# tomdbar/naqs-for-quantum-chemistry

Measured on AMD Instinct MI355X. Metric: unique samples/sec through E_loc + log-psi eval (N2, 20 qubits), higher is better.
Workload: dtype f32 network (f16x2-split MFMA, f32-equivalent) / f64 E_loc; 1 GPU; N2 STO-3G (20 qubits, K=2239 Pauli terms, Kxy=378), 10000 unique samples per GPU, 1xMI355X per rank; pipeline=2 independent batches in flight on 2 HIP streams (one handle pair each), batches=4 distinct key sets per rank, rotated every step, input=unique sampled bit-strings (keys) resident in HBM; random-init network, ranks=single process, no process group

## Files before the change

naqs-for-quantum-chemistry_amd/csrc/naqs_logpsi.hip:

```cpp

#include <algorithm>
#include <cstdint>
#include <cstdio>
#include <cstring>
#include <new>
#include <vector>

#include "naqs_common.hpp"
#include "naqs_hash.hpp"
#include "naqs_net.hpp"
#include "naqs_amp_mfma.hpp"
#include "naqs_amp_deep.hpp"
#include "naqs_pack.hpp"

namespace {

using naqs::WAVE;
using naqs::DeviceGuard;
using naqs::ElocFeed;

using naqs::MAXP;
using naqs::MAXL;
using naqs::f32x4;
using naqs::NetDims;
using naqs::amp_partial;
using naqs::amp_finish;

#ifndef NAQS_AMP_TILES
#define NAQS_AMP_TILES 4
#endif
#ifndef NAQS_AMP_SPLIT
#define NAQS_AMP_SPLIT 4
#endif
constexpr int AMP_TILES = NAQS_AMP_TILES;
constexpr int AMP_SPLIT = NAQS_AMP_SPLIT;

__device__ __forceinline__ void amp_body(const NetDims &d, const float *__restrict__ w, int64_t M,
// ... 1051 lines not shown
                v = mfma_h<2>(a[0][rb], b[0][c], v);
                acc[rb][c] = v;
            }
    };
#pragma unroll
    for (int c0 = 0; c0 < NC; c0 += 2) load_b2(0, c0);
    load_a(0, a0);
    int k0 = 0;
    for (; k0 + 64 <= Kh_pad; k0 += 64) {
        load_a(k0 + 32, a1);
#pragma unroll
        for (int c0 = 0; c0 < NC; c0 += 2) {
            __builtin_amdgcn_sched_barrier(0);
            mma2(a0, c0);
            __builtin_amdgcn_sched_barrier(0);
            load_b2(k0 + 32, c0);
        }
        const int kn = min(k0 + 64, Kh_pad - 32);
        load_a(kn, a0);
#pragma unroll
        for (int c0 = 0; c0 < NC; c0 += 2) {
            __builtin_amdgcn_sched_barrier(0);
            mma2(a1, c0);
            __builtin_amdgcn_sched_barrier(0);
            load_b2(kn, c0);
        }
    }
    if (k0 < Kh_pad) {
#pragma unroll
        for (int c0 = 0; c0 < NC; c0 += 2) mma2(a0, c0);
    }
}

#ifndef NAQS_SAVE_NT
#define NAQS_SAVE_NT 1
#endif
__device__ __forceinline__ void save_store(f32x4 *ptr, const f32x4 val) {
#if NAQS_SAVE_NT
    __builtin_nontemporal_store(val, ptr);
#else
    *ptr = val;
#endif
}
template <int RB, bool SAVE, int NCT, int C0>
__device__ __forceinline__ void ws_writeback4(ushort_t *__restrict__ planes, int ldh, f32x4 (&acc)[RB][NCT],
                                              const float (&bvs)[NCT], int col0, int lane, float *__restrict__ save, int save_ld,
                                              int64_t row0, int64_t M, const LayerScale sc) {
    constexpr int BM = RB * 16;
    const int kg = lane >> 4;
    const int plane_stride = BM * ldh;
#pragma unroll
    for (int rb = 0; rb < RB; ++rb)
#pragma unroll
        for (int r = 0; r < 4; ++r) {
            float h[4];
#pragma unroll
            for (int c = 0; c < 4; ++c) h[c] = fmaxf(fmaf(acc[rb][C0 + c][r], sc.c, bvs[C0 + c]), 0.0f);
            const int row = rb * 16 + kg * 4 + r;
            if (SAVE && save != nullptr && row0 + row < M)
                save_store(reinterpret_cast<f32x4 *>(save + (row0 + row) * save_ld + col0),
                           (f32x4){h[0] * sc.isn, h[1] * sc.isn, h[2] * sc.isn, h[3] * sc.isn});
            ushort_t *dst = planes + row * ldh + col0;
            uint32_t a1, a2, b1, b2;
            split2_pair(h[0], h[1], a1, a2);
            split2_pair(h[2], h[3], b1, b2);
            *reinterpret_cast<uint2 *>(dst) = make_uint2(a1, b1);
// ... 22 lines not shown
            __builtin_amdgcn_sched_barrier(0);
            amp_mfma_item<CT>(d, f0, n, ab, lane, outs);
        } else {
            if (na < n && n_last > n) { na = n + 1; amp_mfma_load<CT>(wamp + (size_t)na * pair_elems, lane, f0); }
            __builtin_amdgcn_sched_barrier(0);
            amp_mfma_item<CT>(d, f1, n, ab, lane, outs);
        }
    }
    if (clk != nullptr && blockIdx.x == 0 && lane == 0) clk[wave * 16 + 8] = clock64();
    {
        const int r = aw * WAVE + lane;
        if (do_feed && r < BM && feed.tab != nullptr && row0 + r < M) {
            const uint64_t key = keys[row0 + r];
            if (feed.key_bits == 32) naqs::feed_key<uint32_t>(feed, row0 + r, key);
            else naqs::feed_key<uint64_t>(feed, row0 + r, key);
        }
    }
    __builtin_amdgcn_fence(__ATOMIC_RELEASE, "wavefront");
    __builtin_amdgcn_wave_barrier();
    __builtin_amdgcn_fence(__ATOMIC_ACQUIRE, "wavefront");
    for (int e = q0 * 16 + lane; e < q1 * 16; e += WAVE) {
        const int q = e >> 4, s = e & 15;
        const int n = q / RB, r = (q - n * RB) * 16 + s;
        float o[5];
#pragma unroll
        for (int c = 0; c < 5; ++c) o[c] = s_o[((size_t)n * BM + r) * 8 + c];
        const uint32_t ab = s_ab[r], mask = (1u << n) - 1u;
        const int occ = (int)((ab >> n) & 1u) + 2 * (int)((ab >> (16 + n)) & 1u);
        s_lan[n][r] = naqs::amp_finish(d, n, o, ab & mask, (ab >> 16) & mask, occ);
    }
    if (clk != nullptr && blockIdx.x == 0 && lane == 0) clk[wave * 16 + 15] = clock64();
}

struct WsSplit {
    unsigned long long *xchg; uint32_t tag; const naqs::PollCtl *ctl;
    const int64_t *spec_U; int spec_P;
    naqs::SampleFinishJob fin;
};
constexpr int WS_XCHG_ROWS = 80;

template <int RB, bool SAVE, bool SPLIT = false>
__global__ __launch_bounds__(PH_THREADS) void phase_kernel_ws(const NetDims d, const float *__restrict__ w,
                                                              const ushort_t *__restrict__ wh, int64_t M,
                                                              const uint64_t *__restrict__ keys,
                                                              const float *__restrict__ scratch, float2 *__restrict__ out,
                                                              const ElocFeed feed, const naqs::PhaseSave save,
                                                              const ushort_t *__restrict__ wamp,
                                                              const naqs::PhaseScales *__restrict__ scales, const int flags,
                                                              const WsSplit split) {
    extern __shared__ __attribute__((aligned(16))) ushort_t planes[];
    __shared__ uint32_t s_ab[RB * 16];
    __shared__ float s_lan[MAXP][RB * 16];
    __shared__ __attribute__((aligned(16))) float s_part[WS_MW][RB * 16][4];
    __shared__ float s_recv[SPLIT ? RB * 16 : 1][4];
    constexpr int BM = RB * 16;
    constexpr int FMT = 2, NP = 2;
    constexpr int AW = PH_WAVES - WS_MW;
    const int tid = threadIdx.x, lane = tid & 63, wave = __builtin_amdgcn_readfirstlane(tid >> 6);
    const int hosted = split.fin.U != nullptr ? 1 : 0;
    if (hosted && blockIdx.x == 0) {
        __shared__ int64_t s_fin[16];
        naqs::sample_finish_body(split.fin, s_fin);
        return;
    }
    const int bx = (int)blockIdx.x - hosted;
    const int n_tiles = SPLIT ? (int)((gridDim.x - hosted) >> 1) : (int)gridDim.x - hosted;
    const bool producer = SPLIT && bx < n_tiles;
    const int tile = SPLIT && !producer ? bx - n_tiles : bx;
    const int64_t row0 = (int64_t)tile * BM;
    if (split.spec_U != nullptr) {
        const int64_t m_dev = split.spec_U[MAXP + 1] != 0 ? 0 : split.spec_U[split.spec_P];
        M = m_dev < M ? m_dev : M;
        if (row0 >= M) return;
    }
    const int P = d.P, ldh = d.ldh;
    float *s_o = reinterpret_cast<float *>(planes + (size_t)NP * BM * ldh);
    const bool ha64 = d.Ha == 64;

    NAQS_MARK(0);
    uint32_t warm0 = 0, warm1 = 0;
    {
        const uint32_t *w0 = reinterpret_cast<const uint32_t *>(wh + d.wh_off[0]);
        const int n_dw = NP * d.N_pad[0] * d.Kh_pad[0] / 2;
        if (tid * 32 < n_dw) warm0 = w0[tid * 32];
        if ((tid + PH_THREADS) * 32 < n_dw) warm1 = w0[(tid + PH_THREADS) * 32];
    }
    static_assert(BM <= WAVE, "the tile's rows are gathered by wave 0");
    uint64_t key = 0ull;
    if (tid < BM && row0 + tid < M) key = keys[row0 + tid];
    const int aw = wave >= WS_MW ? wave - WS_MW : 0;
    const int items = RB * P;
    const int q_split = SPLIT ? (P / 2) * RB : items;
    const int qlo = producer ? q_split : 0, qhi = producer ? items : q_split;
    const int first_pair = (qlo + (qhi - qlo) * aw / AW) / RB;
    AmpFrag<4> f4;
    AmpFrag<2> f2;
    if (wamp != nullptr && wave >= WS_MW) {
        if (ha64) amp_mfma_load<4>(wamp + (size_t)first_pair * amp_mfma_pair_elems(64), lane, f4);
        else amp_mfma_load<2>(wamp + (size_t)first_pair * amp_mfma_pair_elems(32), lane, f2);
    }
    bf16x8 pre[NP][CBT];
    mlp_layer0_fetch<RB, NP>(d, wh + d.wh_off[0], wave, lane, pre);
    if (tid < BM) {
        uint32_t a = 0, b = 0;
#pragma unroll
        for (int k = 0; k < MAXP; ++k) {
            if (k < P) {
                a |= (uint32_t)((key >> d.qa[k]) & 1ull) << k;
                b |= (uint32_t)((key >> d.qb[k]) & 1ull) << k;
            }
        }
        s_ab[tid] = a | (b << 16);
    }
    __syncthreads();
    NAQS_MARK(1);

    const int m = lane & 15, kg = lane >> 4;
    LayerScale sc;
    sc.c = scales->c[0]; sc.sn = scales->sn[0]; sc.isn = scales->isn[0];
    {
        const int N0 = d.N_pad[0], cb0 = wave * CBT;
        float bvs0[CBT];
#pragma unroll
        for (int c = 0; c < CBT; ++c) bvs0[c] = (w + d.b_off[0])[tile_col(cb0 + c, m, N0)] * sc.sn;
        const uint32_t pmask = (1u << (P - 1)) - 1u;
        const int nv = min(max(2 * (P - 1) - 8 * kg, 0), 8) >> 1;
        f32x4 acc0[RB][CBT];
#pragma unroll
        for (int rb = 0; rb < RB; ++rb) {
            const uint32_t ab = s_ab[rb * 16 + m];
// ... 25 lines not shown
                    save.x[(row0 + r) * save.x_ld + k] = set ? 1.0f : -1.0f;
                }
            }
        }
        ws_writeback4<RB, SAVE, CBT, 0>(planes, ldh, acc0, bvs0, (cb0 >> 2) * 64 + 4 * m, lane, producer ? nullptr : save.act[0], save.act_ld[0],
                                        row0, M, sc);
    }
    asm volatile("" ::"v"(warm0), "v"(warm1));
    __syncthreads();
    NAQS_MARK(5);

    sc.c = scales->c[1]; sc.sn = scales->sn[1]; sc.isn = scales->isn[1];
    const int N1 = d.N_pad[1], Kh1 = d.Kh_pad[1];
    if (wave < WS_MW) {
        constexpr int NCT = SPLIT ? WS_NCT / 2 : WS_NCT;
        constexpr int NG = NCT / 4;
        f32x4 acc[RB][NCT];
        float bvs[NCT];
        if (flags & 1) __builtin_amdgcn_s_setprio(1);
#pragma unroll
        for (int rb = 0; rb < RB; ++rb)
#pragma unroll
            for (int c = 0; c < NCT; ++c) acc[rb][c] = (f32x4){0.f, 0.f, 0.f, 0.f};
        const int cb0 = (producer ? WS_MW * NCT : 0) + wave * NCT;
        const float *bias = w + d.b_off[1];
#pragma unroll
        for (int c = 0; c < NCT; ++c) bvs[c] = bias[tile_col(cb0 + c, m, N1)] * sc.sn;
        const ushort_t *a_ptr = planes + m * ldh + 8 * kg, *w_ptr = wh + d.wh_off[1] + (size_t)cb0 * Kh1 * 16 + lane * 8;
        if (flags & 8) {}
#ifdef NAQS_WS_DEBUG
        else if (flags & 16) ws_accumulate<RB, 1, NCT>(a_ptr, ldh, BM * ldh, w_ptr, Kh1, (size_t)N1 * Kh1, acc);
        else if (flags & 32) ws_accumulate<RB, 2, NCT>(a_ptr, ldh, BM * ldh, w_ptr, Kh1, (size_t)N1 * Kh1, acc);
#endif
        else ws_accumulate<RB, 0, NCT>(a_ptr, ldh, BM * ldh, w_ptr, Kh1, (size_t)N1 * Kh1, acc);
        if (flags & 1) __builtin_amdgcn_s_setprio(0);
        NAQS_MARK(9);
        const float *W2 = w + d.w_off[2];
        const int K2 = d.K_pad[2];
        const int g0 = cb0 >> 2;
        f32x4 wv[NG][4];
#pragma unroll
        for (int g = 0; g < NG; ++g)
#pragma unroll
            for (int o = 0; o < 4; ++o) wv[g][o] = *reinterpret_cast<const f32x4 *>(W2 + (size_t)o * K2 + (g0 + g) * 64 + 4 * m);
#pragma unroll
        for (int rb = 0; rb < RB; ++rb)
#pragma unroll
            for (int r = 0; r < 4; ++r) {
                const int row = rb * 16 + kg * 4 + r;
                float po[4] = {0.f, 0.f, 0.f, 0.f};
#pragma unroll
                for (int g = 0; g < NG; ++g) {
                    float h[4];
#pragma unroll
                    for (int c = 0; c < 4; ++c) h[c] = fmaxf(fmaf(acc[rb][4 * g + c][r], sc.c, bvs[4 * g + c]), 0.0f);
                    if (SAVE && save.act[1] != nullptr && row0 + row < M)
                        save_store(reinterpret_cast<f32x4 *>(save.act[1] + (row0 + row) * save.act_ld[1] + (g0 + g) * 64 + 4 * m),
                                   (f32x4){h[0] * sc.isn, h[1] * sc.isn, h[2] * sc.isn, h[3] * sc.isn});
#pragma unroll
                    for (int o = 0; o < 4; ++o)
#pragma unroll
                        for (int c = 0; c < 4; ++c) po[o] = fmaf(h[c], wv[g][o][c], po[o]);
                }
#pragma unroll
                for (int o = 0; o < 4; ++o) {
                    float v = po[o];
                    v += __builtin_bit_cast(float, __builtin_amdgcn_update_dpp(0, __builtin_bit_cast(int, v), 0xB1, 0xF, 0xF, true));
                    v += __builtin_bit_cast(float, __builtin_amdgcn_update_dpp(0, __builtin_bit_cast(int, v), 0x4E, 0xF, 0xF, true));
                    v += __builtin_bit_cast(float, __builtin_amdgcn_update_dpp(0, __builtin_bit_cast(int, v), 0x141, 0xF, 0xF, true));
                    v += __builtin_bit_cast(float, __builtin_amdgcn_update_dpp(0, __builtin_bit_cast(int, v), 0x140, 0xF, 0xF, true));
                    po[o] = v;
                }
                if (m == 0) *reinterpret_cast<f32x4 *>(&s_part[wave][row][0]) = (f32x4){po[0], po[1], po[2], po[3]};
            }
    } else {
        if (flags & 2) __builtin_amdgcn_s_setprio(1);
        if ((flags & 4) || wamp == nullptr) {}
        else if (ha64) ws_amp_work<4, RB>(d, wamp, M, row0, keys, feed, s_ab, s_lan, s_o, f4, aw, lane, save.clk, wave, qlo, qhi, !producer);
        else ws_amp_work<2, RB>(d, wamp, M, row0, keys, feed, s_ab, s_lan, s_o, f2, aw, lane, save.clk, wave, qlo, qhi, !producer);
        if (flags & 2) __builtin_amdgcn_s_setprio(0);
    }
    NAQS_MARK(10);
    __syncthreads();
    NAQS_MARK(6);

    if constexpr (SPLIT) {
        constexpr int TILE_WORDS = BM * 4 + MAXP * BM;
        static_assert(BM <= WS_XCHG_ROWS, "a tile's words must fit the exchange buffer's per-tile share");
        unsigned long long *xw = split.xchg + (size_t)tile * TILE_WORDS;
        const int n_split = q_split / RB, n_amp = wamp != nullptr ? (P - n_split) * BM : 0;
        const unsigned long long tagw = (unsigned long long)split.tag << 32;
        if (producer) {
            for (int x = tid; x < BM * 4 + n_amp; x += PH_THREADS) {
                float v;
                if (x < BM * 4) {
                    const int r = x >> 2, o = x & 3;
                    v = (s_part[0][r][o] + s_part[1][r][o]) + (s_part[2][r][o] + s_part[3][r][o]);
                } else {
                    const int e = x - BM * 4;
                    v = s_lan[n_split + e / BM][e % BM];
                }
                if (!(naqs::poll_drop(split.ctl, naqs::POLL_LOGPSI_SPLIT) && tile == 0 && x == 0))
                    __hip_atomic_store(&xw[x], tagw | __float_as_uint(v), __ATOMIC_RELAXED, __HIP_MEMORY_SCOPE_AGENT);
            }
            return;
        }
        bool ok = true;
        for (int x = tid; x < BM * 4 + n_amp; x += PH_THREADS) {
            unsigned long long word;
            ok = naqs::poll_tagged<2>(&xw[x], split.tag, word, split.ctl, naqs::POLL_LOGPSI_SPLIT, (uint32_t)x) && ok;
// ... 296 lines not shown
    const bool deep = net->amp.deep(), mlp = naqs::has_phase_mlp(net);
    hipDeviceProp_t prop;
    if (hipGetDeviceProperties(&prop, net->device) == hipSuccess) net->cu_count = prop.multiProcessorCount;
    int st = NAQS_OK;
    if (mlp || !deep) st = dev_alloc(&net->d_w, net->w_floats);
    if (st == NAQS_OK && deep) st = dev_alloc(&net->amp.w, net->amp.deep_floats);
    if (!deep) net->amp.w = net->d_w;
    if (st == NAQS_OK && naqs::has_second_set(net)) st = dev_alloc(&net->ph.w, net->ph.deep() ? net->ph.deep_floats : rows_floats(net->ph.d));
    if (st == NAQS_OK && !deep && (d.Ha == 32 || d.Ha == 64 || d.Ha == 128) && (mlp || 2 * (d.P - 1) <= 30))
        st = dev_alloc(&net->d_wamp, (int64_t)d.P * (int64_t)amp_mfma_pair_elems(d.Ha));
    if (st == NAQS_OK && net->family == naqs::Family::COMBINED) st = dev_alloc(&net->d_cflat, net->comb_amp + net->comb_head);
    if (st != NAQS_OK || !mlp) return st;
    st = dev_alloc(&net->d_wh, net->wh_elems);
    if (st != NAQS_OK) return st;
    const int lds_max = 4 * 16 * std::max(d.ld, PH_WAVES * 16) * (int)sizeof(float);
    (void)hipFuncSetAttribute(reinterpret_cast<const void *>(&phase_kernel<1>), hipFuncAttributeMaxDynamicSharedMemorySize, lds_max / 4);
    (void)hipFuncSetAttribute(reinterpret_cast<const void *>(&phase_kernel<2>), hipFuncAttributeMaxDynamicSharedMemorySize, lds_max / 2);
    (void)hipFuncSetAttribute(reinterpret_cast<const void *>(&phase_kernel<3>), hipFuncAttributeMaxDynamicSharedMemorySize, lds_max / 4 * 3);
    (void)hipFuncSetAttribute(reinterpret_cast<const void *>(&phase_kernel<4>), hipFuncAttributeMaxDynamicSharedMemorySize, lds_max);
    const int lds_all = 160 * 1024 - 5 * 1024;
#define NAQS_PH_ATTR(RB, FMT)                                                                                                            \
    (void)hipFuncSetAttribute(reinterpret_cast<const void *>(&phase_kernel_h<RB, false, FMT>), hipFuncAttributeMaxDynamicSharedMemorySize, lds_all); \
    (void)hipFuncSetAttribute(reinterpret_cast<const void *>(&phase_kernel_h<RB, true, FMT>), hipFuncAttributeMaxDynamicSharedMemorySize, lds_all);
    NAQS_PH_ATTR(1, 1) NAQS_PH_ATTR(2, 1) NAQS_PH_ATTR(3, 1)
    NAQS_PH_ATTR(1, 2) NAQS_PH_ATTR(2, 2) NAQS_PH_ATTR(3, 2) NAQS_PH_ATTR(4, 2)
#undef NAQS_PH_ATTR
#define NAQS_WS_ATTR(RB)                                                                                                                 \
    (void)hipFuncSetAttribute(reinterpret_cast<const void *>(&phase_kernel_ws<RB, false>), hipFuncAttributeMaxDynamicSharedMemorySize, lds_all); \
    (void)hipFuncSetAttribute(reinterpret_cast<const void *>(&phase_kernel_ws<RB, true>), hipFuncAttributeMaxDynamicSharedMemorySize, lds_all); \
    (void)hipFuncSetAttribute(reinterpret_cast<const void *>(&phase_kernel_ws<RB, false, true>), hipFuncAttributeMaxDynamicSharedMemorySize, lds_all); \
    (void)hipFuncSetAttribute(reinterpret_cast<const void *>(&phase_kernel_ws<RB, true, true>), hipFuncAttributeMaxDynamicSharedMemorySize, lds_all);
    NAQS_WS_ATTR(1) NAQS_WS_ATTR(2) NAQS_WS_ATTR(3)
#undef NAQS_WS_ATTR
    (void)hipGetLastError();
    st = dev_alloc(&net->d_raw, 1);
    if (st == NAQS_OK) st = dev_alloc(&net->d_scales, 1);
    if (st == NAQS_OK && hipMemset(net->d_raw, 0, sizeof(naqs::PhaseRaw)) != hipSuccess) st = NAQS_ERR_HIP;
    if (st == NAQS_OK) st = dev_alloc(&net->d_sum_words, 8);
    if (st == NAQS_OK && hipMemset(net->d_sum_words, 0, 8 * sizeof(unsigned long long)) != hipSuccess) st = NAQS_ERR_HIP;
    if (st == NAQS_OK && hipDeviceSynchronize() != hipSuccess) st = NAQS_ERR_HIP;
    return st;
}

static int net_build(const naqs_net_config_t *cfg, const naqs::Family family, const int depth, const int device, naqs_net_t **out) {
    int st = net_validate(cfg, family, depth, device);
    if (st != NAQS_OK) return st;
    naqs_net *net = new (std::nothrow) naqs_net();
    if (!net) return NAQS_ERR_NOMEM;
    net->device = device;
    net->cfg = *cfg;
    net->family = family;
    st = net_layout(net, depth);
    if (st != NAQS_OK) { delete net; return st; }
    (void)naqs::poll_handle_create(device, &net->poll);
    net->ctl = net->poll.dev;
    net->shared_gpu = naqs::env_int("NAQS_SHARED_GPU", 0) == 1;
    DeviceGuard guard;
    st = guard.init(device);
    if (st == NAQS_OK) st = net_alloc(net);
    if (st != NAQS_OK) { naqs_net_destroy(net); return st; }
    *out = net;
    return NAQS_OK;
}

NAQS_API int naqs_net_create(const naqs_net_config_t *cfg, int device, naqs_net_t **out) {
    if (!cfg || !out) return NAQS_ERR_INVALID;
// ... 469 lines not shown
        const ElocFeed none{};
        if (prof) { st = net->prof.begin(s); if (st != NAQS_OK) return st; }
        st = launch_amp_kernel(net->ph.d, net->ph.w, M, keys_dev, s_ph, none, 1, s);
        if (st != NAQS_OK) return st;
        if (prof) { st = net->prof.end(s); if (st != NAQS_OK) return st; }
    }
    NAQS_KLAUNCH(agg_finish_kernel, dim3((unsigned)((M + 255) / 256)), dim3(256), 0, s, net->amp.d.P, M, net->d_scratch, s_ph,
                       reinterpret_cast<float2 *>(logpsi_dev), feed);
    HIP_TRY(hipGetLastError());
    return NAQS_OK;
}

static int comb_logpsi(naqs_net *net, int64_t M, const uint64_t *keys_dev, float *logpsi_dev, hipStream_t s, const ElocFeed &feed) {
    const NetDims &d = net->amp.d, &dh = net->ph.d;
    const bool prof = net->prof.armed();
    if (prof) { int stp = net->prof.begin(s); if (stp != NAQS_OK) return stp; }
    int st = naqs::net_amp_forward(net, M, keys_dev, s, &feed);
    if (st != NAQS_OK) return st;
    float *s_head = net->d_scratch + (size_t)d.P * net->cap_M;
    const size_t lds = (size_t)naqs::amp_block_floats(dh.Ha, 2 * (dh.P - 1)) * sizeof(float);
    if (lds > 64 * 1024) return NAQS_ERR_UNSUPPORTED;
    NAQS_KLAUNCH(comb_head_kernel, dim3((unsigned)((M + AMP_TILES * WAVE - 1) / (AMP_TILES * WAVE)), (unsigned)dh.P),
                       dim3(AMP_TILES * AMP_SPLIT * WAVE), lds, s, dh, net->ph.w, M, keys_dev, s_head);
    HIP_TRY(hipGetLastError());
    NAQS_KLAUNCH(comb_finish_kernel, dim3((unsigned)((M + 255) / 256)), dim3(256), 0, s, d.P, M, net->d_scratch,
                       s_head + (size_t)(dh.P - 1) * M, reinterpret_cast<float2 *>(logpsi_dev), feed);
    HIP_TRY(hipGetLastError());
    if (prof) { st = net->prof.end(s); if (st != NAQS_OK) return st; }
    std::snprintf(net->last_kernel, sizeof(net->last_kernel), "%s + comb_head_kernel + comb_finish_kernel", net->last_amp);
    return NAQS_OK;
}

struct FormSel { bool ws = false, ws_split = false; int rb = 1; };
static FormSel select_form(const naqs_net *net, const int64_t M, const int fmt, const size_t lds_h16, const int rb_max) {
    const NetDims &d = net->amp.d;
    FormSel f;
    const bool ws_shape = fmt == 2 && d.n_lin == 3 && d.N_pad[0] == PH_WAVES * CBT * 16 && d.N_pad[1] == WS_MW * WS_NCT * 16 &&
                          d.Kh_pad[0] == 32 && d.N_pad[2] == 16 && (d.Ha == 64 || d.Ha == 32) && CBT == 4 && PH_WAVES == 8;
    const int ws_mode = naqs::env_int("NAQS_PHASE_WS", 1);
    int rb = naqs::env_int("NAQS_PHASE_RB", 0);
    if (rb < 1 || rb > rb_max) rb = (int)std::min<int64_t>(rb_max, std::max<int64_t>(1, (M + 16ll * net->cu_count - 1) / (16ll * net->cu_count)));
    bool ws = ws_shape && ws_mode != 0 && !d.phase_sym;
    if (ws) {
        const int rb_ws = std::min(rb, 3);
        if (rb_ws * lds_h16 + (size_t)d.P * rb_ws * 16 * 8 * sizeof(float) > 155 * 1024) ws = false;
        else rb = rb_ws;
    }
    bool ws_split = false;
    if (ws && naqs::env_int("NAQS_WS_SPLIT", 1) != 0) {
        int rbs = naqs::env_int("NAQS_WS_SPLIT_RB", 0);
        if (rbs < 1 || rbs > 3) rbs = 1;
        const int64_t tiles = (M + 16 * rbs - 1) / (16 * rbs);
        if (2 * tiles <= net->cu_count && rbs * lds_h16 + (size_t)d.P * rbs * 16 * 8 * sizeof(float) <= 155 * 1024) { ws_split = true; rb = rbs; }
    }
    f.ws = ws; f.ws_split = ws_split; f.rb = rb;
    return f;
}

naqs::PhaseForm naqs::net_logpsi_form(const naqs_net *net, const int64_t M) {
    PhaseForm f;
    const NetDims &d = net->amp.d;
    if (!naqs::has_phase_mlp(net)) return f;
    const int fmt = phase_format(d);
    if (fmt == 0) return f;
    const size_t lds_h16 = phase_slab_bytes(d, fmt);
    const int rb_max = phase_rb_max(d, fmt);
    const size_t amp_scratch = (size_t)d.P * rb_max * 16 * 8 * sizeof(float);
    const bool amp_in_phase = net->d_wamp != nullptr && net->wamp_fresh && naqs::env_int("NAQS_AMP_MODE", 1) == 1 &&
                              amp_scratch <= 150 * 1024 && d.Ha <= 64;
    const FormSel sel = select_form(net, M, fmt, lds_h16, rb_max);
    f.kind = (sel.ws && amp_in_phase) ? 1 : 0; f.rb = sel.rb; f.split = sel.ws_split ? 1 : 0;
    return f;
}

int naqs::net_logpsi_impl(naqs_net *net, int64_t M, const uint64_t *keys_dev, float *logpsi_dev, void *stream,
                          const ElocFeed &feed, const PhaseSave &save, const SpecRows *spec) {
    if (!net || M < 0 || (M > 0 && (!keys_dev || !logpsi_dev))) return NAQS_ERR_INVALID;
    if (!net->have_weights) return NAQS_ERR_INVALID;
    if (M == 0) return NAQS_OK;
    if (M >= (1ll << 31)) return NAQS_ERR_UNSUPPORTED;
    DeviceGuard guard;
    int st = guard.init(net->device);
    if (st != NAQS_OK) return st;
    st = naqs::poll_check(net->poll);
    if (st != NAQS_OK) return st;
    const NetDims &d = net->amp.d;
    hipStream_t s = reinterpret_cast<hipStream_t>(stream);
    st = naqs::net_flush_pack(net, s);
    if (st != NAQS_OK) return st;
    switch (net->family) {
        case naqs::Family::AGGREGATE:
            return net->amp.deep() ? agg_deep_logpsi(net, M, keys_dev, logpsi_dev, s, feed) : agg_logpsi(net, M, keys_dev, logpsi_dev, s, feed);
        case naqs::Family::COMBINED: return comb_logpsi(net, M, keys_dev, logpsi_dev, s, feed);
        case naqs::Family::SINGLE_PHASE: break;
    }
    const int fmt = phase_format(d);
    if (fmt != net->packed_fmt) return NAQS_ERR_INVALID;
    const bool use_h = fmt != 0;
    const size_t lds_h16 = use_h ? phase_slab_bytes(d, fmt) : 0;
    const int rb_max = phase_rb_max(d, fmt);
    const size_t amp_scratch = (size_t)d.P * rb_max * 16 * 8 * sizeof(float);
    const bool amp_in_phase = use_h && net->d_wamp != nullptr && net->wamp_fresh && naqs::env_int("NAQS_AMP_MODE", 1) == 1 &&
                              amp_scratch <= 150 * 1024 && d.Ha <= 64;
    if (spec && !(amp_in_phase && save.x != nullptr && select_form(net, spec->m_var, fmt, lds_h16, rb_max).ws)) return NAQS_ERR_UNSUPPORTED;
    if (!amp_in_phase) {
        st = naqs::net_amp_forward(net, M, keys_dev, s, &feed);
        if (st != NAQS_OK) return st;
    }
    const unsigned short *wamp = amp_in_phase ? net->d_wamp : nullptr;
    naqs::PhaseSave save_dbg = save;
    long long *clk_dev = nullptr;
    if (naqs::env_int("NAQS_DEBUG_CLOCKS", 0) == 1) {
        HIP_TRY(hipMalloc((void **)&clk_dev, 128 * sizeof(long long)));
        HIP_TRY(hipMemset(clk_dev, 0, 128 * sizeof(long long)));
        save_dbg.clk = clk_dev;
    }

    if (save.x != nullptr && !use_h) return NAQS_ERR_UNSUPPORTED;
    if (!use_h && !net->packed_f32) return NAQS_ERR_INVALID;
    const FormSel sel = select_form(net, spec ? spec->m_var : M, fmt, lds_h16, rb_max);
    const bool ws = sel.ws, ws_split = sel.ws_split;
    const int rb = sel.rb;
    const int bm = rb * 16;
    const unsigned grid = (unsigned)((M + bm - 1) / bm);
    const size_t ksplit_scratch = (size_t)PH_WAVES * bm * 16 * sizeof(float);
    float2 *out = reinterpret_cast<float2 *>(logpsi_dev);
    WsSplit split{nullptr, 0u, net->ctl, spec ? spec->U : nullptr, spec ? spec->P : 0, naqs::SampleFinishJob{}};
    const bool host_fin = spec && spec->host_finish && net->fin_pending;
    if (host_fin) split.fin = net->fin_job;
    const unsigned hosted = host_fin ? 1u : 0u;
    if (ws_split) {
        const size_t tiles_cap = std::max<size_t>((size_t)(net->cu_count / 2), (size_t)grid);
        const size_t words = tiles_cap * (WS_XCHG_ROWS * 4 + MAXP * WS_XCHG_ROWS);
        if (net->d_ws_xchg && net->ws_xchg_words < words) {
            HIP_TRY(hipDeviceSynchronize());
            (void)hipFree(net->d_ws_xchg);
            net->d_ws_xchg = nullptr;
        }
        net->ws_xchg_words = std::max(net->ws_xchg_words, words);
        if (!net->d_ws_xchg) {
            HIP_TRY(hipMalloc((void **)&net->d_ws_xchg, net->ws_xchg_words * sizeof(unsigned long long)));
            HIP_TRY(hipMemset(net->d_ws_xchg, 0, net->ws_xchg_words * sizeof(unsigned long long)));
            HIP_TRY(hipDeviceSynchronize());
            net->ws_seq = 0;
        }
        if (++net->ws_seq == 0u) {
            HIP_TRY(hipMemsetAsync(net->d_ws_xchg, 0, net->ws_xchg_words * sizeof(unsigned long long), s));
            net->ws_seq = 1u;
        }
        split.xchg = net->d_ws_xchg;
        split.tag = net->ws_seq;
    }
    net->last_form_kind = (ws && amp_in_phase) ? 1 : 0; net->last_form_rb = rb; net->last_form_split = ws_split ? 1 : 0;
    const bool prof = net->prof.armed();
    if (prof) { st = net->prof.begin(s); if (st != NAQS_OK) return st; }
    if (ws) std::snprintf(net->last_kernel, sizeof(net->last_kernel), "phase_kernel_ws<RB=%d, SAVE=%d%s> (f16x2%s)", rb,
                          save.x != nullptr ? 1 : 0, ws_split ? ", SPLIT=1" : "", amp_in_phase ? ", amplitude waves beside the matrix waves" : "");
    else if (use_h) std::snprintf(net->last_kernel, sizeof(net->last_kernel), "phase_kernel_h<RB=%d, SAVE=%d, FMT=%d (%s)>%s", rb, save.x != nullptr ? 1 : 0,
                             fmt, fmt == 2 ? "f16x2" : "bf16x3", amp_in_phase ? " incl. amplitude prologue" : "");
    else std::snprintf(net->last_kernel, sizeof(net->last_kernel), "phase_kernel<RB=%d> (f32 MFMA)", rb);
    if (!amp_in_phase) {
        const size_t n = std::strlen(net->last_kernel);
        std::snprintf(net->last_kernel + n, sizeof(net->last_kernel) - n, " + %s", net->last_amp);
    }
    if (ws) {
        const size_t lds = rb * lds_h16 + (size_t)d.P * bm * 8 * sizeof(float);
        const int flags = naqs::env_int("NAQS_WS_FLAGS", 0);
#define NAQS_WS_LAUNCH(RB)                                                                                                              \
        do {                                                                                                                            \
            if (save.x != nullptr) NAQS_KLAUNCH((phase_kernel_ws<RB, true>), dim3(grid + hosted), dim3(PH_THREADS), lds, s, d, net->d_w, net->d_wh, M, keys_dev, net->d_scratch, out, feed, save_dbg, wamp, net->d_scales, flags, split); \
            else NAQS_KLAUNCH((phase_kernel_ws<RB, false>), dim3(grid + hosted), dim3(PH_THREADS), lds, s, d, net->d_w, net->d_wh, M, keys_dev, net->d_scratch, out, feed, save_dbg, wamp, net->d_scales, flags, split); \
        } while (0)
#define NAQS_WS_LAUNCH_SPLIT(RB)                                                                                                        \
        do {                                                                                                                            \
            if (save.x != nullptr) NAQS_KLAUNCH((phase_kernel_ws<RB, true, true>), dim3(2 * grid + hosted), dim3(PH_THREADS), lds, s, d, net->d_w, net->d_wh, M, keys_dev, net->d_scratch, out, feed, save_dbg, wamp, net->d_scales, flags, split); \
            else NAQS_KLAUNCH((phase_kernel_ws<RB, false, true>), dim3(2 * grid + hosted), dim3(PH_THREADS), lds, s, d, net->d_w, net->d_wh, M, keys_dev, net->d_scratch, out, feed, save_dbg, wamp, net->d_scales, flags, split); \
        } while (0)
        if (ws_split) {
            switch (rb) {
                case 1: NAQS_WS_LAUNCH_SPLIT(1); break;
                case 2: NAQS_WS_LAUNCH_SPLIT(2); break;
                default: NAQS_WS_LAUNCH_SPLIT(3); break;
            }
        } else {
            switch (rb) {
                case 1: NAQS_WS_LAUNCH(1); break;
                case 2: NAQS_WS_LAUNCH(2); break;
                default: NAQS_WS_LAUNCH(3); break;
            }
        }
#undef NAQS_WS_LAUNCH_SPLIT
#undef NAQS_WS_LAUNCH
        if (hosted) net->fin_pending = false;
    } else if (use_h) {
        const size_t lds = std::max(std::max(rb * lds_h16, amp_in_phase ? amp_scratch : (size_t)0), ksplit_scratch);
#define NAQS_PH_LAUNCH(RB, FMT)                                                                                                         \
        do {                                                                                                                            \
            if (save.x != nullptr) NAQS_KLAUNCH((phase_kernel_h<RB, true, FMT>), dim3(grid), dim3(PH_THREADS), lds, s, d, net->d_w, net->d_wh, M, keys_dev, net->d_scratch, out, feed, save_dbg, wamp, net->d_scales); \
            else NAQS_KLAUNCH((phase_kernel_h<RB, false, FMT>), dim3(grid), dim3(PH_THREADS), lds, s, d, net->d_w, net->d_wh, M, keys_dev, net->d_scratch, out, feed, save_dbg, wamp, net->d_scales); \
        } while (0)
        if (fmt == 2) {
            switch (rb) {
                case 1: NAQS_PH_LAUNCH(1, 2); break;
                case 2: NAQS_PH_LAUNCH(2, 2); break;
                case 3: NAQS_PH_LAUNCH(3, 2); break;
                default: NAQS_PH_LAUNCH(4, 2); break;
            }
        } else {
            switch (rb) {
                case 1: NAQS_PH_LAUNCH(1, 1); break;
                case 2: NAQS_PH_LAUNCH(2, 1); break;
                default: NAQS_PH_LAUNCH(3, 1); break;
            }
        }
#undef NAQS_PH_LAUNCH
    } else {
        const size_t lds = std::max((size_t)bm * d.ld * sizeof(float), ksplit_scratch);
        switch (rb) {
            case 1: NAQS_KLAUNCH(phase_kernel<1>, dim3(grid), dim3(PH_THREADS), lds, s, d, net->d_w, M, keys_dev, net->d_scratch, out, feed); break;
            case 2: NAQS_KLAUNCH(phase_kernel<2>, dim3(grid), dim3(PH_THREADS), lds, s, d, net->d_w, M, keys_dev, net->d_scratch, out, feed); break;
            case 3: NAQS_KLAUNCH(phase_kernel<3>, dim3(grid), dim3(PH_THREADS), lds, s, d, net->d_w, M, keys_dev, net->d_scratch, out, feed); break;
// ... 89 lines not shown
```

Baseline: 357.3 million unique samples/s.

## Deduplicate shared-prefix amplitude evaluations in warp-specialized phase kernel

Adds a dedup path to the amplitude waves. Rows in a tile whose occupation prefix up to orbital n matches the previous row share the conditional-amplitude evaluation: ballot/mbcnt finds distinct runs per orbital and only unique runs go through the MFMA, with results scattered back per row. This is enabled by default through NAQS_AMP_DEDUP. It also adds an opt-in RB=4 variant with a ring-buffered weight-prefetch accumulator, and an LDS-fit check that now counts the kernel's static shared memory. The gain depends on sorted keys sharing prefixes, and the change adds extra LDS, barriers and bookkeeping.

```diff
diff --git a/naqs-for-quantum-chemistry_amd/csrc/naqs_logpsi.hip b/naqs-for-quantum-chemistry_amd/csrc/naqs_logpsi.hip
--- a/naqs-for-quantum-chemistry_amd/csrc/naqs_logpsi.hip
+++ b/naqs-for-quantum-chemistry_amd/csrc/naqs_logpsi.hip
@@ -3,6 +3,7 @@
 #include <cstdint>
 #include <cstdio>
 #include <cstring>
+#include <mutex>
 #include <new>
 #include <vector>
 
@@ -1120,6 +1121,57 @@
     }
 }
 
+constexpr int WS_RING4 = 6;
+constexpr int ws_lcm(int a, int b) { int x = a; while (x % b != 0) x += a; return x; }
+template <int RB, int NC, int SL>
+__device__ __forceinline__ void ws_accumulate_ring(const ushort_t *__restrict__ a_ptr, int ldh, int plane_stride,
+                                                   const ushort_t *__restrict__ w_ptr, int Kh_pad, size_t wplane,
+                                                   f32x4 (&acc)[RB][NC]) {
+    static_assert(SL <= NC, "the ring is filled from the first chunk");
+    constexpr int PER = ws_lcm(NC, SL), CPB = PER / NC;
+    bf16x8 b[SL][2], a[2][RB];
+    const int k_last = Kh_pad - 32;
+    auto load_b = [&](int slot, int k, int c) {
+#pragma unroll
+        for (int p = 0; p < 2; ++p) b[slot][p] = *reinterpret_cast<const bf16x8 *>(w_ptr + p * wplane + ((size_t)c * Kh_pad + k) * 16);
+    };
+    auto load_a = [&](int k, int rb) {
+#pragma unroll
+        for (int p = 0; p < 2; ++p) a[p][rb] = *reinterpret_cast<const bf16x8 *>(a_ptr + p * plane_stride + rb * 16 * ldh + k);
+    };
+    auto step = [&](int t, int k0) {
+        const int ch = t / NC, c = t % NC, slot = t % SL;
+        __builtin_amdgcn_sched_barrier(0);
+#pragma unroll
+        for (int rb = 0; rb < RB; ++rb) {
+            f32x4 v = acc[rb][c];
+            v = mfma_h<2>(a[1][rb], b[slot][0], v);
+            v = mfma_h<2>(a[0][rb], b[slot][1], v);
+            v = mfma_h<2>(a[0][rb], b[slot][0], v);
+            acc[rb][c] = v;
+            if (c == NC - 1) load_a(min(k0 + 32 * (ch + 1), k_last), rb);
+        }
+        __builtin_amdgcn_sched_barrier(0);
+        load_b(slot, min(k0 + 32 * ((t + SL) / NC), k_last), (t + SL) % NC);
+    };
+#pragma unroll
+    for (int t = 0; t < SL; ++t) load_b(t, 0, t);
+#pragma unroll
+    for (int rb = 0; rb < RB; ++rb) load_a(0, rb);
+    int k0 = 0;
+    for (; k0 + 32 * CPB <= Kh_pad; k0 += 32 * CPB) {
+#pragma unroll
+        for (int t = 0; t < PER; ++t) step(t, k0);
+    }
+#pragma unroll
+    for (int ch = 0; ch < CPB - 1; ++ch) {
+        if (k0 + 32 * ch < Kh_pad) {
+#pragma unroll
+            for (int c = 0; c < NC; ++c) step(ch * NC + c, k0);
+        }
+    }
+}
+
 #ifndef NAQS_SAVE_NT
 #define NAQS_SAVE_NT 1
 #endif
@@ -1208,11 +1260,134 @@
     if (clk != nullptr && blockIdx.x == 0 && lane == 0) clk[wave * 16 + 15] = clock64();
 }
 
+constexpr int WS_FLAG_DEDUP = 64;
+constexpr int WS_DD_ITEMS = 16;
+struct WsDedupLds {
+    uint32_t ab[PH_WAVES - WS_MW][16];
+    uint32_t item[PH_WAVES - WS_MW][WS_DD_ITEMS];
+};
+static_assert(4 * MAXP <= (PH_WAVES - WS_MW) * WS_DD_ITEMS, "an amplitude wave's items must fit WsDedupLds::item");
+
+template <int CT, int RB>
+__device__ __forceinline__ void ws_amp_work_dedup(const NetDims &d, const ushort_t *__restrict__ wamp, int64_t M, int64_t row0,
+                                                  const uint64_t *__restrict__ keys, const ElocFeed &feed, const uint32_t *s_ab,
+                                                  float (*s_lan)[RB * 16], float *__restrict__ s_o, WsDedupLds &dd, int aw, int lane,
+                                                  long long *clk, int wave, int nlo, int nhi, bool do_feed) {
+    constexpr int BM = RB * 16;
+    constexpr int AW = PH_WAVES - WS_MW;
+    const size_t pair_elems = amp_mfma_pair_elems(CT * 16);
+    uint32_t ab_row = 0u;
+    int h = 99;
+    if (lane < BM) {
+        ab_row = s_ab[lane];
+        const uint32_t x = ab_row ^ s_ab[lane > 0 ? lane - 1 : 0];
+        const uint32_t x16 = (x | (x >> 16)) & 0xFFFFu;
+        h = x16 != 0u ? __builtin_ctz(x16) : 32;
+        if (row0 + lane >= M) h = 32;
+        if (lane == 0) h = -1;
+    }
+    auto runs_of = [&](int n) -> unsigned long long { return __builtin_amdgcn_ballot_w64(h < n); };
+    auto run_of = [&](unsigned long long B, int n) -> int {
+        const int below = (int)__builtin_amdgcn_mbcnt_hi((uint32_t)(B >> 32), __builtin_amdgcn_mbcnt_lo((uint32_t)B, 0u));
+        return below + (h < n ? 1 : 0) - 1;
+    };
+    int total = 0;
+    for (int n = nlo; n < nhi; ++n) total += (__builtin_popcountll(runs_of(n)) + 15) >> 4;
+    const int q0 = total * aw / AW, q1 = total * (aw + 1) / AW;
+    int n = nlo, j = 0;
+    unsigned long long B = 0ull;
+    int D = 0, cnt = 0;
+    if (q0 < q1) {
+        int before = 0;
+        for (;; ++n) {
+            B = runs_of(n);
+            D = __builtin_popcountll(B);
+            cnt = (D + 15) >> 4;
+            if (q0 < before + cnt) break;
+            before += cnt;
+        }
+        j = q0 - before;
+    }
+    AmpFrag<CT> f0, f1;
+    if (q0 < q1) amp_mfma_load<CT>(wamp + (size_t)n * pair_elems, lane, f0);
+    bool in0 = true;
+    bool entered = true;
+    for (int q = q0; q < q1; ++q) {
+        const int run = run_of(B, n);
+        if (h < n && (run >> 4) == j) dd.ab[aw][run & 15] = ab_row;
+        __builtin_amdgcn_fence(__ATOMIC_RELEASE, "wavefront");
+        __builtin_amdgcn_wave_barrier();
+        __builtin_amdgcn_fence(__ATOMIC_ACQUIRE, "wavefront");
+        const int s = lane & 15, last = min(D - 16 * j, 16) - 1;
+        const uint32_t ab = dd.ab[aw][min(s, last)];
+        float *outs = s_o + ((size_t)n * BM + j * 16) * 8;
+        const bool more = entered && q + (cnt - j) < q1;
+        entered = false;
+        if (in0) {
+            if (more) amp_mfma_load<CT>(wamp + (size_t)(n + 1) * pair_elems, lane, f1);
+            __builtin_amdgcn_sched_barrier(0);
+            amp_mfma_item<CT>(d, f0, n, ab, lane, outs);
+        } else {
+            if (more) amp_mfma_load<CT>(wamp + (size_t)(n + 1) * pair_elems, lane, f0);
+            __builtin_amdgcn_sched_barrier(0);
+            amp_mfma_item<CT>(d, f1, n, ab, lane, outs);
+        }
+        if (lane < 16) outs[s * 8 + 7] = __uint_as_float(ab);
+        if (lane == 0) dd.item[aw][q - q0] = (uint32_t)n | ((uint32_t)j << 8) | ((uint32_t)D << 16);
+        if (++j == cnt && q + 1 < q1) {
+            ++n; j = 0; in0 = !in0; entered = true;
+            B = runs_of(n);
+            D = __builtin_popcountll(B);
+            cnt = (D + 15) >> 4;
+        }
+    }
+    if (clk != nullptr && blockIdx.x == 0 && lane == 0) clk[wave * 16 + 8] = clock64();
+    {
+        const int r = aw * WAVE + lane;
+        if (do_feed && r < BM && feed.tab != nullptr && row0 + r < M) {
+            const uint64_t key = keys[row0 + r];
+            if (feed.key_bits == 32) naqs::feed_key<uint32_t>(feed, row0 + r, key);
+            else naqs::feed_key<uint64_t>(feed, row0 + r, key);
+        }
+    }
+    __builtin_amdgcn_fence(__ATOMIC_RELEASE, "wavefront");
+    __builtin_amdgcn_wave_barrier();
+    __builtin_amdgcn_fence(__ATOMIC_ACQUIRE, "wavefront");
+    for (int e = lane; e < (q1 - q0) * 16; e += WAVE) {
+        const uint32_t it = dd.item[aw][e >> 4];
+        const int ni = (int)(it & 0xFFu), run = (int)((it >> 8) & 0xFFu) * 16 + (e & 15);
+        if (run < (int)(it >> 16)) {
+            float *os = s_o + ((size_t)ni * BM + run) * 8;
+            float o[5], la[4];
+            bool ok[4];
+#pragma unroll
+            for (int c = 0; c < 5; ++c) o[c] = os[c];
+            const uint32_t ab = __float_as_uint(os[7]), mask = (1u << ni) - 1u;
+            naqs::amp_conditional(d, ni, o, ab & mask, (ab >> 16) & mask, la, ok);
+            *reinterpret_cast<f32x4 *>(os) = (f32x4){la[0], la[1], la[2], la[3]};
+        }
+    }
+    __builtin_amdgcn_fence(__ATOMIC_RELEASE, "wavefront");
+    __builtin_amdgcn_wave_barrier();
+    __builtin_amdgcn_fence(__ATOMIC_ACQUIRE, "wavefront");
+    for (int i = 0; i < q1 - q0; ++i) {
+        const uint32_t it = (uint32_t)__builtin_amdgcn_readfirstlane((int)dd.item[aw][i]);
+        const int ni = (int)(it & 0xFFu), ji = (int)((it >> 8) & 0xFFu);
+        const int run = run_of(runs_of(ni), ni);
+        if (lane < BM && (run >> 4) == ji) {
+            const int occ = (int)((ab_row >> ni) & 1u) + 2 * (int)((ab_row >> (16 + ni)) & 1u);
+            s_lan[ni][lane] = s_o[((size_t)ni * BM + run) * 8 + occ];
+        }
+    }
+    if (clk != nullptr && blockIdx.x == 0 && lane == 0) clk[wave * 16 + 15] = clock64();
+}
+
 struct WsSplit {
     unsigned long long *xchg; uint32_t tag; const naqs::PollCtl *ctl;
     const int64_t *spec_U; int spec_P;
     naqs::SampleFinishJob fin;
 };
+constexpr size_t WS_LDS_LIMIT = 160 * 1024;
 constexpr int WS_XCHG_ROWS = 80;
 
 template <int RB, bool SAVE, bool SPLIT = false>
@@ -1229,9 +1404,11 @@
     __shared__ float s_lan[MAXP][RB * 16];
     __shared__ __attribute__((aligned(16))) float s_part[WS_MW][RB * 16][4];
     __shared__ float s_recv[SPLIT ? RB * 16 : 1][4];
+    __shared__ WsDedupLds s_dd;
     constexpr int BM = RB * 16;
     constexpr int FMT = 2, NP = 2;
     constexpr int AW = PH_WAVES - WS_MW;
+    const bool dedup = (flags & WS_FLAG_DEDUP) != 0;
     const int tid = threadIdx.x, lane = tid & 63, wave = __builtin_amdgcn_readfirstlane(tid >> 6);
     const int hosted = split.fin.U != nullptr ? 1 : 0;
     if (hosted && blockIdx.x == 0) {
@@ -1271,7 +1448,7 @@
     const int first_pair = (qlo + (qhi - qlo) * aw / AW) / RB;
     AmpFrag<4> f4;
     AmpFrag<2> f2;
-    if (wamp != nullptr && wave >= WS_MW) {
+    if (wamp != nullptr && wave >= WS_MW && !dedup) {
         if (ha64) amp_mfma_load<4>(wamp + (size_t)first_pair * amp_mfma_pair_elems(64), lane, f4);
         else amp_mfma_load<2>(wamp + (size_t)first_pair * amp_mfma_pair_elems(32), lane, f2);
     }
@@ -1363,6 +1540,7 @@
         else if (flags & 16) ws_accumulate<RB, 1, NCT>(a_ptr, ldh, BM * ldh, w_ptr, Kh1, (size_t)N1 * Kh1, acc);
         else if (flags & 32) ws_accumulate<RB, 2, NCT>(a_ptr, ldh, BM * ldh, w_ptr, Kh1, (size_t)N1 * Kh1, acc);
 #endif
+        else if constexpr (RB == 4) ws_accumulate_ring<RB, NCT, WS_RING4>(a_ptr, ldh, BM * ldh, w_ptr, Kh1, (size_t)N1 * Kh1, acc);
         else ws_accumulate<RB, 0, NCT>(a_ptr, ldh, BM * ldh, w_ptr, Kh1, (size_t)N1 * Kh1, acc);
         if (flags & 1) __builtin_amdgcn_s_setprio(0);
         NAQS_MARK(9);
@@ -1407,6 +1585,11 @@
     } else {
         if (flags & 2) __builtin_amdgcn_s_setprio(1);
         if ((flags & 4) || wamp == nullptr) {}
+        else if (dedup) {
+            const int n_lo = producer ? P / 2 : 0, n_hi = SPLIT && !producer ? P / 2 : P;
+            if (ha64) ws_amp_work_dedup<4, RB>(d, wamp, M, row0, keys, feed, s_ab, s_lan, s_o, s_dd, aw, lane, save.clk, wave, n_lo, n_hi, !producer);
+            else ws_amp_work_dedup<2, RB>(d, wamp, M, row0, keys, feed, s_ab, s_lan, s_o, s_dd, aw, lane, save.clk, wave, n_lo, n_hi, !producer);
+        }
         else if (ha64) ws_amp_work<4, RB>(d, wamp, M, row0, keys, feed, s_ab, s_lan, s_o, f4, aw, lane, save.clk, wave, qlo, qhi, !producer);
         else ws_amp_work<2, RB>(d, wamp, M, row0, keys, feed, s_ab, s_lan, s_o, f2, aw, lane, save.clk, wave, qlo, qhi, !producer);
         if (flags & 2) __builtin_amdgcn_s_setprio(0);
@@ -1769,6 +1952,7 @@
     (void)hipFuncSetAttribute(reinterpret_cast<const void *>(&phase_kernel_ws<RB, true, true>), hipFuncAttributeMaxDynamicSharedMemorySize, lds_all);
     NAQS_WS_ATTR(1) NAQS_WS_ATTR(2) NAQS_WS_ATTR(3)
 #undef NAQS_WS_ATTR
+    (void)hipFuncSetAttribute(reinterpret_cast<const void *>(&phase_kernel_ws<4, false>), hipFuncAttributeMaxDynamicSharedMemorySize, lds_all);
     (void)hipGetLastError();
     st = dev_alloc(&net->d_raw, 1);
     if (st == NAQS_OK) st = dev_alloc(&net->d_scales, 1);
@@ -2304,27 +2488,51 @@
 }
 
 struct FormSel { bool ws = false, ws_split = false; int rb = 1; };
-static FormSel select_form(const naqs_net *net, const int64_t M, const int fmt, const size_t lds_h16, const int rb_max) {
+static size_t ws_static_lds(const int rb, const bool split) {
+    static size_t bytes[5][2];
+    static std::once_flag once;
+    std::call_once(once, [] {
+        const void *fn[5][2] = {{nullptr, nullptr},
+                                {reinterpret_cast<const void *>(&phase_kernel_ws<1, false>), reinterpret_cast<const void *>(&phase_kernel_ws<1, false, true>)},
+                                {reinterpret_cast<const void *>(&phase_kernel_ws<2, false>), reinterpret_cast<const void *>(&phase_kernel_ws<2, false, true>)},
+                                {reinterpret_cast<const void *>(&phase_kernel_ws<3, false>), reinterpret_cast<const void *>(&phase_kernel_ws<3, false, true>)},
+                                {reinterpret_cast<const void *>(&phase_kernel_ws<4, false>), nullptr}};
+        for (int r = 1; r <= 4; ++r)
+            for (int sp = 0; sp < 2; ++sp) {
+                hipFuncAttributes at;
+                bytes[r][sp] = fn[r][sp] != nullptr && hipFuncGetAttributes(&at, fn[r][sp]) == hipSuccess ? at.sharedSizeBytes : WS_LDS_LIMIT;
+            }
+        (void)hipGetLastError();
+    });
+    return bytes[rb][split ? 1 : 0];
+}
+static bool ws_lds_fits(const NetDims &d, const int rb, const bool split, const size_t lds_h16) {
+    return rb * lds_h16 + (size_t)d.P * rb * 16 * 8 * sizeof(float) + ws_static_lds(rb, split) <= WS_LDS_LIMIT;
+}
+static FormSel select_form(const naqs_net *net, const int64_t M, const int fmt, const size_t lds_h16, const int rb_max, const bool save) {
     const NetDims &d = net->amp.d;
     FormSel f;
     const bool ws_shape = fmt == 2 && d.n_lin == 3 && d.N_pad[0] == PH_WAVES * CBT * 16 && d.N_pad[1] == WS_MW * WS_NCT * 16 &&
                           d.Kh_pad[0] == 32 && d.N_pad[2] == 16 && (d.Ha == 64 || d.Ha == 32) && CBT == 4 && PH_WAVES == 8;
     const int ws_mode = naqs::env_int("NAQS_PHASE_WS", 1);
-    int rb = naqs::env_int("NAQS_PHASE_RB", 0);
+    const int rb_env = naqs::env_int("NAQS_PHASE_RB", 0);
+    int rb = rb_env;
     if (rb < 1 || rb > rb_max) rb = (int)std::min<int64_t>(rb_max, std::max<int64_t>(1, (M + 16ll * net->cu_count - 1) / (16ll * net->cu_count)));
     bool ws = ws_shape && ws_mode != 0 && !d.phase_sym;
     if (ws) {
         const int rb_ws = std::min(rb, 3);
-        if (rb_ws * lds_h16 + (size_t)d.P * rb_ws * 16 * 8 * sizeof(float) > 155 * 1024) ws = false;
+        if (!ws_lds_fits(d, rb_ws, false, lds_h16)) ws = false;
         else rb = rb_ws;
     }
+    const bool rb4 = ws && !save && rb_max >= 4 && rb_env == 4 && ws_lds_fits(d, 4, false, lds_h16);
     bool ws_split = false;
     if (ws && naqs::env_int("NAQS_WS_SPLIT", 1) != 0) {
         int rbs = naqs::env_int("NAQS_WS_SPLIT_RB", 0);
         if (rbs < 1 || rbs > 3) rbs = 1;
         const int64_t tiles = (M + 16 * rbs - 1) / (16 * rbs);
-        if (2 * tiles <= net->cu_count && rbs * lds_h16 + (size_t)d.P * rbs * 16 * 8 * sizeof(float) <= 155 * 1024) { ws_split = true; rb = rbs; }
-    }
+        if (2 * tiles <= net->cu_count && ws_lds_fits(d, rbs, true, lds_h16)) { ws_split = true; rb = rbs; }
+    }
+    if (rb4) { rb = 4; ws_split = false; }
     f.ws = ws; f.ws_split = ws_split; f.rb = rb;
     return f;
 }
@@ -2340,7 +2548,7 @@
     const size_t amp_scratch = (size_t)d.P * rb_max * 16 * 8 * sizeof(float);
     const bool amp_in_phase = net->d_wamp != nullptr && net->wamp_fresh && naqs::env_int("NAQS_AMP_MODE", 1) == 1 &&
                               amp_scratch <= 150 * 1024 && d.Ha <= 64;
-    const FormSel sel = select_form(net, M, fmt, lds_h16, rb_max);
+    const FormSel sel = select_form(net, M, fmt, lds_h16, rb_max, true);
     f.kind = (sel.ws && amp_in_phase) ? 1 : 0; f.rb = sel.rb; f.split = sel.ws_split ? 1 : 0;
     return f;
 }
@@ -2374,7 +2582,7 @@
     const size_t amp_scratch = (size_t)d.P * rb_max * 16 * 8 * sizeof(float);
     const bool amp_in_phase = use_h && net->d_wamp != nullptr && net->wamp_fresh && naqs::env_int("NAQS_AMP_MODE", 1) == 1 &&
                               amp_scratch <= 150 * 1024 && d.Ha <= 64;
-    if (spec && !(amp_in_phase && save.x != nullptr && select_form(net, spec->m_var, fmt, lds_h16, rb_max).ws)) return NAQS_ERR_UNSUPPORTED;
+    if (spec && !(amp_in_phase && save.x != nullptr && select_form(net, spec->m_var, fmt, lds_h16, rb_max, true).ws)) return NAQS_ERR_UNSUPPORTED;
     if (!amp_in_phase) {
         st = naqs::net_amp_forward(net, M, keys_dev, s, &feed);
         if (st != NAQS_OK) return st;
@@ -2390,7 +2598,7 @@
 
     if (save.x != nullptr && !use_h) return NAQS_ERR_UNSUPPORTED;
     if (!use_h && !net->packed_f32) return NAQS_ERR_INVALID;
-    const FormSel sel = select_form(net, spec ? spec->m_var : M, fmt, lds_h16, rb_max);
+    const FormSel sel = select_form(net, spec ? spec->m_var : M, fmt, lds_h16, rb_max, save.x != nullptr);
     const bool ws = sel.ws, ws_split = sel.ws_split;
     const int rb = sel.rb;
     const int bm = rb * 16;
@@ -2437,7 +2645,7 @@
     }
     if (ws) {
         const size_t lds = rb * lds_h16 + (size_t)d.P * bm * 8 * sizeof(float);
-        const int flags = naqs::env_int("NAQS_WS_FLAGS", 0);
+        const int flags = (naqs::env_int("NAQS_WS_FLAGS", 0) & ~WS_FLAG_DEDUP) | (naqs::env_int("NAQS_AMP_DEDUP", 1) != 0 ? WS_FLAG_DEDUP : 0);
 #define NAQS_WS_LAUNCH(RB)                                                                                                              \
         do {                                                                                                                            \
             if (save.x != nullptr) NAQS_KLAUNCH((phase_kernel_ws<RB, true>), dim3(grid + hosted), dim3(PH_THREADS), lds, s, d, net->d_w, net->d_wh, M, keys_dev, net->d_scratch, out, feed, save_dbg, wamp, net->d_scales, flags, split); \
@@ -2458,7 +2666,10 @@
             switch (rb) {
                 case 1: NAQS_WS_LAUNCH(1); break;
                 case 2: NAQS_WS_LAUNCH(2); break;
-                default: NAQS_WS_LAUNCH(3); break;
+                case 3: NAQS_WS_LAUNCH(3); break;
+                default:
+                    NAQS_KLAUNCH((phase_kernel_ws<4, false>), dim3(grid + hosted), dim3(PH_THREADS), lds, s, d, net->d_w, net->d_wh, M, keys_dev, net->d_scratch, out, feed, save_dbg, wamp, net->d_scales, flags, split);
+                    break;
             }
         }
 #undef NAQS_WS_LAUNCH_SPLIT
```

Measured after the change: 360.7 million unique samples/s, median of 6. About the same (+0.9%).
